# compbioproj-cdna-to-genome-map-align/gmap-2024

Measured on AMD Instinct MI355X. Metric: aligned cDNA reads/sec (2 kb, GRCh38) at 1/2/4/8 MI355X; DP HBM GB/s vs peak, higher is better.
Workload: dtype int32

## Files before the change

gmap-2024_amd/csrc/gmapdp_engine.cpp:

```cpp
#include <dlfcn.h>
#include <hip/hip_runtime.h>
#include <time.h>
#include <unistd.h>

#include <algorithm>
#include <climits>
#include <cctype>
#include <cstdio>
#include <cstdlib>
#include <cstring>
#include <map>
#include <memory>
#include <condition_variable>
#include <mutex>
#include <thread>
#include <atomic>
#include <sys/mman.h>
#include <string>
#include <tuple>
#include <utility>
#include <vector>

#include "gmapdp_internal.h"
#include "me_device.h"
// ... 841 lines not shown
  if (!T) return GMAPDP_EINVAL;
  hipError_t e = ctx->din.ensure(16 * n);
  if (e == hipSuccess) e = ctx->dout.ensure(n);
  if (e != hipSuccess) return fail(ctx, GMAPDP_ENOMEM, "canonical-link buffers: %s", e);
  unsigned char* din = (unsigned char*)ctx->din.p;
  hipStream_t s = ctx->stream;
  e = hipMemcpyAsync(din, prevpos, 8 * n, hipMemcpyHostToDevice, s);
  if (e == hipSuccess) e = hipMemcpyAsync(din + 8 * n, currpos, 8 * n, hipMemcpyHostToDevice, s);
  if (e == hipSuccess)
    e = launch_canon_links((long long)n, s, ctx->d_genome, ctx->genome_words, T, (const gmapdp_coord_t*)din,
                           (const gmapdp_coord_t*)(din + 8 * n), plusp, chroffset, chrhigh, (uint8_t*)ctx->dout.p);
  if (e == hipSuccess) e = hipMemcpyAsync(out, ctx->dout.p, n, hipMemcpyDeviceToHost, s);
  if (e == hipSuccess) e = ctx_sync(ctx, s);
  return e == hipSuccess ? GMAPDP_OK : fail(ctx, GMAPDP_ELAUNCH, "canonical links: %s", e);
}

}

static const size_t kLdsBudget = 64 * 1024;
static size_t env_size(const char* name, size_t dflt);
static size_t dpx_lds_dirs_max() {
  static const size_t v = env_size("GMAPDP_DPX_LDS_DIRS_MAX", 4 * 1024);
  return v;
}

static int pick_R(int W) {
  int R = 1;
  while (R * 64 < W) R <<= 1;
  return R;
}

static size_t lds_bucket(size_t lds) {
  static const size_t b[] = {4096, 8192, 16384, 32768, 49152, 65536, 98304, 163840};
  for (size_t x : b)
    if (lds <= x) return x;
  return lds;
}

static size_t gg_lds_bucket(size_t lds) {
  static const size_t b[] = {4096,  6144,  8192,  10240, 12288, 14336, 16384, 20480, 24576,
                             28672, 32768, 40960, 49152, 65536, 98304, 163840};
  for (size_t x : b)
    if (lds <= x) return x;
  return lds;
}

static size_t env_size(const char* name, size_t dflt) {
  const char* e = getenv(name);
  return e ? (size_t)strtoull(e, nullptr, 10) : dflt;
}

static size_t gg_lds_dirs_max() { return env_size("GMAPDP_GG_LDS_DIRS_MAX", 0); }
static bool gg_rowfill() { return env_size("GMAPDP_GG_ROWFILL", 1) != 0; }
static bool rows_disabled() {
  static const bool v = env_size("GMAPDP_DP_ROWS", 1) == 0;
  return v;
}
static size_t latency_batch() {
  static const size_t v = env_size("GMAPDP_LATENCY_BATCH", 1024);
  return v;
}

static size_t slot_bucket(size_t b) {
  static const size_t s[] = {256, 384, 512, 768, 1024, 1536, 2048, 3072, 4096, 6144, 8192, 12288, 16384};
  for (size_t x : s)
    if (b <= x) return x;
  return 0;
}

static void null_result(gmapdp_result& res, int score, int dpi) {
  res.npairs = 0;
  res.traceback_score = score;
  res.nmatches = res.nmismatches = res.nopens = res.nindels = 0;
  res.dynprogindex = dpi;
}

static int next_dpi(int dpi) { return dpi + (dpi > 0 ? 1 : -1); }

static int convert_single(const gmapdp_ctx* ctx, const gmapdp_single_problem& p, gmapdp_result& res, DevProblem& d) {
  if (p.rlength <= 0 || p.glength <= 0 || p.rlength > GMAPDP_MAX_RLENGTH || p.glength > GMAPDP_MAX_GLENGTH) {
    null_result(res, GMAPDP_NEG_INFINITY_32, next_dpi(p.dynprogindex));
    return 0;
  }
  std::memset(&d, 0, sizeof(d));
  d.kind = kSingle;
  d.qbase = p.qoff;
  d.rlength = p.rlength;
  d.glength = p.glength;
  d.roffset = p.roffset;
  d.goffset = p.goffset;
  d.chroffset = p.chroffset;
  d.chrhigh = p.chrhigh;
  const double dr = p.defect_rate;
  d.mismatchtype = dr < 0.003 ? kHighQ : (dr < 0.014 ? kMedQ : kLowQ);
  if (ctx->user_dynprog_p) {
    d.open = ctx->user_open;
    d.extend = ctx->user_extend;
  } else if (dr < 0.003) {
    d.open = -8; d.extend = -3;
  } else if (dr < 0.014) {
    d.open = -7; d.extend = -2;
  } else {
    d.open = -6; d.extend = -1;
  }
  const bool watson = p.flags & GMAPDP_WATSON;
  d.flags = (watson ? kFWatson : 0) | ((p.flags & GMAPDP_JUMP_LATE) ? kFLate : 0) |
// ... 1903 lines not shown
struct OligoClasses {
  std::vector<int> key;
  std::vector<size_t> slots;
  std::map<int, std::vector<int>> classes;
};
static const int kBuckets[] = {1024, 2048, 4096, 8192, 16384};

static int oligo_classify(gmapdp_ctx* ctx, const gmapdp_oligo_problem* problems, int n, const char* qseq_uc,
                          size_t qbytes, bool major_only, OligoClasses& C) {
  std::vector<int> distinct(n, 0);
  std::vector<const char*> rej(n, nullptr);
  plan_parallel((size_t)n, plan_threads((size_t)n * 128), [&](size_t lo, size_t hi, int) {
    std::vector<uint32_t> bm(2048, 0u);
    for (size_t i = lo; i < hi; i++) {
      const gmapdp_oligo_problem& p = problems[i];
      if (major_only && p.minor)
        rej[i] = "Stage2_scan takes the major oligoindex only (minor must be 0)";
      else if (p.querylength <= 8)
        rej[i] = "stage-2 seeding needs querylength > 8 (Oligoindex_set_inquery)";
      else if (p.qoff < 0 || (size_t)p.qoff + (size_t)p.querylength > qbytes)
        rej[i] = "query outside the arena";
      else
        distinct[i] = oligo_distinct(qseq_uc + p.qoff, p.querylength, bm);
    }
  });
  C.key.resize(n);
  C.slots.resize(n);
  for (int i = 0; i < n; i++) {
    const gmapdp_oligo_problem& p = problems[i];
    if (rej[i]) return bad(ctx, rej[i]);
    const uint64_t win = oligo_window(p);
    if (win > 0) {
      const uint64_t lpl = (uint64_t)p.chroffset + p.chrend + (p.plusp ? 0 : 1) - 8;
      const uint64_t h = (lpl >> 4) + 1;
      if (3 * (h >> 1) + 1 >= ctx->genome_words) return bad(ctx, "stage-2 window past the genome");
    }
    if (distinct[i] > kOligoMaxDistinct && !ctx->long_queries)
      return bad(ctx, "query with more than 16384 distinct 8-mers");
    if (distinct[i] > kOligoMaxDistinct) {
      C.key[i] = kOligoLongKey;
      ctx->long_calls.fetch_add(1, std::memory_order_relaxed);
    } else {
      int umax = kBuckets[0];
      for (int b : kBuckets)
        if (distinct[i] <= b) { umax = b; break; }
      C.key[i] = 2 * umax + (win >= 65536 ? 1 : 0);
    }
    C.slots[i] = oligo_pool_slots(p);
    C.classes[C.key[i]].push_back(i);
  }
  return GMAPDP_OK;
}

static void oligo_dev_problem(DevOligoProblem& d, const gmapdp_oligo_problem& p, int umax, int mode) {
  std::memset(&d, 0, sizeof(d));
  d.querylength = p.querylength;
  d.chrstart = p.chrstart;
  d.chrend = p.chrend;
  d.chroffset = p.chroffset;
  d.chrhigh = p.chrhigh;
  d.plusp = p.plusp ? 1 : 0;
  d.minor = p.minor ? 1 : 0;
  d.umax = umax;
  d.reduce = oi_reduction_of(mode, p.plusp != 0);
}

extern "C" {

size_t gmapdp_oligo_positions_capacity(const gmapdp_oligo_problem* problems, int n) {
  size_t c = 0;
  for (int i = 0; i < n; i++) c += oligo_table_cap(problems[i]);
  return c;
}
size_t gmapdp_oligo_diagonal_capacity(const gmapdp_oligo_problem* problems, int n) {
  size_t c = 0;
  for (int i = 0; i < n; i++) c += oligo_diag_cap(problems[i]);
  return c;
}

}

struct gmapdp_oligo_plan {
  int n = 0;
  DevMem<DevOligoProblem> d_probs;
  DevMem<unsigned char> d_scratch;
  std::vector<std::pair<int, int>> launches;
  std::vector<int> umax;
  std::vector<int> keys;
  size_t table_cap = 0, diag_cap = 0, scratch_cap = 0;
  DevMem<int32_t> d_nhits;
  bool split = false;
  DevMem<uint64_t> d_pool;
  DevMem<unsigned long long> d_pool_counter;
  unsigned long long pool_cap = 0;
  bool sizing = false;
  std::vector<DevOligoProblem> ord;
  int mode = 0;
};

static constexpr int kOligoChunkProblems = 16384;
static constexpr size_t kOligoChunkBytes = size_t(3) << 30;
static constexpr size_t kOligoSizingChunkBytes = size_t(32) << 30;

static void oligo_layout(gmapdp_oligo_plan* P, const std::vector<size_t>& slots, bool fallback,
                         const std::vector<size_t>& tcap, const std::vector<size_t>& dcap, bool local,
                         const std::vector<size_t>* hcap = nullptr) {
  P->launches.clear();
  P->umax.clear();
  P->scratch_cap = 0;
  P->pool_cap = 0;
  P->table_cap = 0;
  P->diag_cap = 0;
  size_t cb = 0, cs = 0, ct = 0, cd = 0;
  int first = 0;
  auto close = [&](int end) {
    if (end > first) {
      P->launches.push_back({first, end - first});
// ... 33 lines not shown
}

static hipError_t oligo_buffers(gmapdp_ctx* ctx, gmapdp_oligo_plan* P) {
  const int n = P->n;
  hipError_t e = hipSuccess;
  if (P->split || P->sizing) {
    const bool t = P->sizing;
    e = ctx->oprobs.ensure(sizeof(DevOligoProblem) * std::max(n, 1));
    if (e == hipSuccess) e = ctx->oscratch.ensure(std::max<size_t>(P->scratch_cap, 256), t);
    if (e == hipSuccess) e = ctx->opool.ensure(sizeof(uint64_t) * std::max<size_t>(P->pool_cap, 1), t);
    if (e == hipSuccess) e = ctx->opoolctr.ensure(sizeof(unsigned long long));
    P->d_probs.view((DevOligoProblem*)ctx->oprobs.p);
    P->d_scratch.view((unsigned char*)ctx->oscratch.p);
    P->d_pool.view((uint64_t*)ctx->opool.p);
    P->d_pool_counter.view((unsigned long long*)ctx->opoolctr.p);
    if (e == hipSuccess && n)
      e = hipMemcpyAsync(P->d_probs, P->ord.data(), sizeof(DevOligoProblem) * n, hipMemcpyHostToDevice, ctx->stream);
    return e;
  }
  P->d_scratch.reset();
  P->d_pool.reset();
  if (!P->d_probs.owns()) e = P->d_probs.alloc(sizeof(DevOligoProblem) * std::max(n, 1));
  if (e == hipSuccess) e = P->d_scratch.alloc(std::max<size_t>(P->scratch_cap, 256));
  if (e == hipSuccess) e = P->d_pool.alloc(sizeof(uint64_t) * std::max<size_t>(P->pool_cap, 1));
  if (e == hipSuccess && !P->d_pool_counter.owns()) e = P->d_pool_counter.alloc(sizeof(unsigned long long));
  if (e == hipSuccess && n)
    e = hipMemcpy(P->d_probs, P->ord.data(), sizeof(DevOligoProblem) * n, hipMemcpyHostToDevice);
  return e;
}

static int oligo_plan_build(gmapdp_ctx* ctx, const gmapdp_oligo_problem* problems, int n, const char* qseq_uc,
                            size_t qbytes, std::unique_ptr<gmapdp_oligo_plan>& plan, bool split,
                            bool sizing = false) {
  plan.reset();
  if (const int rc_alt = refuse_alt(ctx, "stage-2 seeding (gmapdp_oligo_*, gmapdp_stage2_*)")) return rc_alt;
  if (oi_reduction_of(ctx->mode, true) < 0)
    return bad(ctx, "stage 2 in a non-stranded cmet / atoi / ttoc mode (GMAP supports the stranded modes only)");
  if (!ctx->d_genome) return GMAPDP_ENOGENOME;
  (void)hipSetDevice(ctx->device);
  OligoClasses C;
  if (int rc = oligo_classify(ctx, problems, n, qseq_uc, qbytes, false, C)) return rc;
  std::vector<size_t> tcap(n), dcap(n);
  for (int i = 0; i < n; i++) {
    tcap[i] = oligo_table_cap(problems[i]);
    dcap[i] = oligo_diag_cap(problems[i]);
  }
  std::unique_ptr<gmapdp_oligo_plan> P(new gmapdp_oligo_plan());
  P->n = n;
  P->mode = ctx->mode;
  P->split = split;
  P->sizing = sizing;
  P->ord.resize(n);
  P->keys.reserve(n);
  for (auto& kv : C.classes)
    for (int i : kv.second) {
      DevOligoProblem& d = P->ord[P->keys.size()];
      oligo_dev_problem(d, problems[i], kv.first >> 1, ctx->mode);
      d.qoff = problems[i].qoff;
      d.index = i;
      P->keys.push_back(kv.first);
    }
  oligo_layout(P.get(), C.slots, !sizing, tcap, dcap, sizing);
  if (const char* ev = std::getenv("GMAPDP_OLIGO_POOL_SLOTS")) P->pool_cap = std::strtoull(ev, nullptr, 10);
  const hipError_t e = oligo_buffers(ctx, P.get());
  if (e != hipSuccess) return fail(ctx, GMAPDP_ENOMEM, "oligo plan: %s", e);
  plan = std::move(P);
  return GMAPDP_OK;
}

static hipError_t oligo_plan_relayout(gmapdp_ctx* ctx, gmapdp_oligo_plan* P, const gmapdp_oligo_problem* problems,
                                      const gmapdp_oligo_result* ores, const int32_t* nhits) {
  const int n = P->n;
  std::vector<size_t> slots(n), tcap(n), dcap(n), hcap(n);
  for (int i = 0; i < n; i++) {
    const size_t tp = (size_t)std::max(ores[i].totalpositions, 0);
    tcap[i] = std::min<size_t>(oligo_table_cap(problems[i]), tp);
    dcap[i] = ores[i].oned_matrix_p < 0 ? oligo_diag_cap(problems[i]) : (size_t)std::max(ores[i].ndiagonals, 0);
    slots[i] = 3 * tp;
    hcap[i] = (size_t)std::max(nhits[i], 0);
  }
  {
    std::vector<int> key(n), idx(n);
    for (int k = 0; k < n; k++) {
      const int i = P->ord[k].index;
      key[k] = (P->keys[k] & 1) && !oligo_key_long(P->keys[k]) && nhits[i] >= 0 && nhits[i] < 65536 ? P->keys[k] - 1
                                                                                                     : P->keys[k];
      idx[k] = k;
    }
    std::stable_sort(idx.begin(), idx.end(), [&](int a, int b) { return key[a] < key[b]; });
    std::vector<DevOligoProblem> ord(n);
    std::vector<int> keys(n);
    for (int k = 0; k < n; k++) {
      ord[k] = P->ord[idx[k]];
      keys[k] = key[idx[k]];
    }
    P->ord.swap(ord);
    P->keys.swap(keys);
  }
  oligo_layout(P, slots, false, tcap, dcap, false, &hcap);
  P->sizing = false;
  P->d_nhits.reset();
  return oligo_buffers(ctx, P);
}

extern "C" {

int gmapdp_oligo_plan_create(gmapdp_ctx* ctx, const gmapdp_oligo_problem* problems, int n, const char* qseq_uc,
                             size_t qbytes, gmapdp_oligo_plan** plan) {
  if (!ctx || !plan || n < 0 || (n > 0 && (!problems || !qseq_uc))) return GMAPDP_EINVAL;
  std::unique_ptr<gmapdp_oligo_plan> p;
// ... 90 lines not shown
  }
  e = hipMemcpyAsync(results, ctx->oresults.p, sizeof(gmapdp_oligo_result) * n, hipMemcpyDeviceToHost, s);
  if (e == hipSuccess) e = hipMemcpyAsync(npositions, ctx->onpos.p, sizeof(int32_t) * qbytes, hipMemcpyDeviceToHost, s);
  if (e == hipSuccess) e = hipMemcpyAsync(mappings, ctx->omap.p, sizeof(int32_t) * qbytes, hipMemcpyDeviceToHost, s);
  if (e == hipSuccess && toff)
    e = hipMemcpyAsync(positions, ctx->otable.p, sizeof(uint32_t) * toff, hipMemcpyDeviceToHost, s);
  if (e == hipSuccess && doff)
    e = hipMemcpyAsync(diagonals, ctx->odiag.p, 4 * sizeof(int32_t) * doff, hipMemcpyDeviceToHost, s);
  if (e == hipSuccess) e = ctx_sync(ctx, s);
  if (e != hipSuccess) return fail(ctx, GMAPDP_ELAUNCH, "oligo execution: %s", e);
  oligo_absolute_mappings(problems, n, results, mappings);
  return GMAPDP_OK;
}

}

struct ScanLaunch {
  int first = 0, count = 0, key = 0;
  unsigned long long pool_slots = 0;
  size_t scratch = 0, pool = 0, table = 0, diag = 0, quc = 0, npos = 0, map = 0, ores = 0, total = 0;
};
struct gmapdp_scan_plan {
  int n = 0, mode = 0;
  DevMem<DevOligoProblem> d_probs;
  DevMem<unsigned char> d_extra;
  DevMem<unsigned char> d_arena;
  size_t arena_bytes = 0, budget = 0;
  std::vector<ScanLaunch> launches;
};

static constexpr size_t kScanBudgetFloor = size_t(8) << 30;

static size_t scan_budget(gmapdp_ctx* ctx) {
  if (const char* ev = std::getenv("GMAPDP_SCAN_ARENA_MB")) return (size_t)std::strtoull(ev, nullptr, 10) << 20;
  size_t held = 0;
  for (const DevBuf* b : {&ctx->oscratch, &ctx->opool, &ctx->otable, &ctx->odiag, &ctx->onpos, &ctx->omap})
    held += b->cap;
  return std::max(held, kScanBudgetFloor);
}

extern "C" {

int gmapdp_scan_plan_create(gmapdp_ctx* ctx, const gmapdp_oligo_problem* problems, int n, const char* qseq_uc,
                            size_t qbytes, gmapdp_scan_plan** plan) {
  if (!ctx || !plan || n < 0 || (n > 0 && (!problems || !qseq_uc))) return GMAPDP_EINVAL;
  *plan = nullptr;
  if (oi_reduction_of(ctx->mode, true) < 0)
    return bad(ctx, "stage 2 in a non-stranded cmet / atoi / ttoc mode (GMAP supports the stranded modes only)");
  if (const int rc_alt = refuse_alt(ctx, "Stage2_scan (gmapdp_scan_plan_*)")) return rc_alt;
  if (!ctx->d_genome) return GMAPDP_ENOGENOME;
  (void)hipSetDevice(ctx->device);
  OligoClasses C;
  if (int rc = oligo_classify(ctx, problems, n, qseq_uc, qbytes,  true, C)) return rc;
  std::unique_ptr<gmapdp_scan_plan> P(new gmapdp_scan_plan());
  P->n = n;
  P->mode = ctx->mode;
  P->budget = scan_budget(ctx);
  struct Extra { int32_t src_qoff, out_index; };
  std::vector<DevOligoProblem> ord;
  std::vector<Extra> extra;
  ord.reserve(n);
  extra.reserve(n);
  size_t cs = 0, cp = 0, ct = 0, cd = 0, cq = 0;
  ScanLaunch L;
  auto close = [&]() {
    if (L.count == 0) return;
    size_t off = 0;
    auto carve = [&](size_t bytes) { const size_t at = off; off = align_up(off + bytes, 256); return at; };
    L.scratch = carve(cs);
    L.pool = carve(sizeof(uint64_t) * cp);
    L.table = carve(sizeof(uint32_t) * ct);
    L.diag = carve(4 * sizeof(int32_t) * cd);
    L.quc = carve(cq);
    L.npos = carve(sizeof(int32_t) * cq);
    L.map = carve(sizeof(int32_t) * cq);
    L.ores = carve(sizeof(gmapdp_oligo_result) * (size_t)L.count);
    L.total = off;
    L.pool_slots = cp;
    P->arena_bytes = std::max(P->arena_bytes, off);
    P->launches.push_back(L);
    L = ScanLaunch();
    L.first = (int)ord.size();
    cs = cp = ct = cd = cq = 0;
  };
  for (auto& kv : C.classes)
    for (int i : kv.second) {
      const gmapdp_oligo_problem& p = problems[i];
      const uint32_t w = p.chrend > p.chrstart ? p.chrend - p.chrstart : 0;
      const size_t lt = oligo_key_long(kv.first) ? scratch_bytes_oi_long() : 0;
      const size_t mb = lt + align_up(scratch_bytes_oi(p.querylength, w), 256);
      const size_t fb = align_up(scratch_bytes_oi_fallback(p.querylength, w), 256);
      const size_t tcap = oligo_table_cap(p), dcap = oligo_diag_cap(p);
      const size_t slots = C.slots[i];
      const size_t qpad = align_up((size_t)p.querylength, 16);
      const size_t bytes = mb + fb + 8 * slots + 4 * tcap + 16 * dcap + 9 * qpad + sizeof(gmapdp_oligo_result) + 8 * 256;
      const size_t open = cs + 8 * cp + 4 * ct + 16 * cd + 9 * cq + sizeof(gmapdp_oligo_result) * (size_t)L.count + 8 * 256;
      if (L.count > 0 && (kv.first != L.key || L.count >= kOligoChunkProblems || open + bytes > P->budget ||
                          cq + qpad > 0x7fffffffull))
        close();
      if (L.count == 0) L.key = kv.first;
      DevOligoProblem d;
      oligo_dev_problem(d, p, kv.first >> 1, ctx->mode);
      d.qoff = (int32_t)cq;
      d.index = L.count;
      d.table_offset = (int64_t)ct;
      d.diag_offset = (int64_t)cd;
      d.scratch_offset = (int64_t)(cs + lt);
      d.fallback_offset = (int64_t)(cs + mb);
      d.hit_cap = (uint32_t)std::min<size_t>((size_t)w + 2, 0xffffffffu);
      d.table_cap = (uint32_t)std::min<size_t>(tcap, 0xffffffffu);
      d.diag_cap = (uint32_t)std::min<size_t>(dcap, 0xffffffffu);
      ord.push_back(d);
      extra.push_back(Extra{p.qoff, i});
      cs += mb + fb;
      cp += slots;
      ct += tcap;
      cd += dcap;
      cq += qpad;
      L.count++;
    }
  close();
  hipError_t e = hipSuccess;
  if (n) {
    e = P->d_probs.alloc(sizeof(DevOligoProblem) * (size_t)n);
    if (e == hipSuccess) e = P->d_extra.alloc(sizeof(Extra) * (size_t)n);
    if (e == hipSuccess) e = P->d_arena.alloc(P->arena_bytes + 256);
    if (e == hipSuccess) e = hipMemcpy(P->d_probs, ord.data(), sizeof(DevOligoProblem) * (size_t)n, hipMemcpyHostToDevice);
    if (e == hipSuccess) e = hipMemcpy(P->d_extra, extra.data(), sizeof(Extra) * (size_t)n, hipMemcpyHostToDevice);
  }
  if (e != hipSuccess) return fail(ctx, GMAPDP_ENOMEM, "scan plan: %s", e);
  *plan = P.release();
  return GMAPDP_OK;
}

int gmapdp_scan_plan_nlaunches(const gmapdp_scan_plan* plan) { return plan ? (int)plan->launches.size() : 0; }
size_t gmapdp_scan_plan_scratch_bytes(const gmapdp_scan_plan* plan) { return plan ? plan->arena_bytes : 0; }
void gmapdp_scan_plan_destroy(gmapdp_scan_plan* plan) { delete plan; }

int gmapdp_scan_plan_run(gmapdp_ctx* ctx, const gmapdp_scan_plan* plan, const char* d_qseq_uc,
                         gmapdp_scan_result* d_results, void* stream) {
  if (!ctx || !plan) return GMAPDP_EINVAL;
  if (const int rc_alt = refuse_alt(ctx, "Stage2_scan (gmapdp_scan_plan_*)")) return rc_alt;
  if (plan->mode != ctx->mode) return bad(ctx, "a scan plan made by a context of another mode");
  if (plan->n == 0) return GMAPDP_OK;
  if (!d_qseq_uc || !d_results) return GMAPDP_EINVAL;
  (void)hipSetDevice(ctx->device);
  hipStream_t s = stream_of(ctx, stream);
  unsigned char* A = plan->d_arena;
  unsigned long long* pool_counter = reinterpret_cast<unsigned long long*>(A + plan->arena_bytes);
  int32_t* flag = reinterpret_cast<int32_t*>(A + plan->arena_bytes + 64);
  if (hipMemsetAsync(flag, 0, sizeof(int32_t), s) != hipSuccess)
    return fail(ctx, GMAPDP_ELAUNCH, "scan flag reset: %s", hipGetLastError());
  for (const ScanLaunch& L : plan->launches) {
    const hipError_t e = launch_s2scan(
        L.key & 1, plan->mode != 0, oligo_key_long(L.key), L.count, lds_bytes_oi(L.key >> 1, L.key & 1), s, plan->d_probs + L.first,
// ... 964 lines not shown
```

gmap-2024_amd/csrc/gmapdp_internal.h:

```cpp
#pragma once
#include <stdint.h>

namespace gmapdp {

constexpr int kNegInf32 = -32768;
constexpr int kMatch = 1, kMismatch = -3, kQopen = -3, kQindel = -1, kTopen = -3, kTindel = -1;
constexpr int kMicrointronLength = 9;
constexpr int kMaxR = 64;

enum GClass : uint8_t { kA = 0, kC = 1, kG = 2, kT = 3, kN = 4, kStar = 5 };
constexpr int kNClass = 8;

enum Kind : int32_t { kSingle = 0, kEnd5 = 1, kEnd3 = 2 };
enum Endalign : int32_t { kQueryendGap = 0, kQueryendIndels = 1, kQueryendNogaps = 2, kBestLocal = 3 };

constexpr int32_t kFWatson = 0x1;
constexpr int32_t kFLate = 0x2;
constexpr int32_t kFRequirePos = 0x4;
constexpr int32_t kFSegLeft = 0x8;
constexpr int32_t kFSegRevcomp = 0x10;
constexpr int32_t kFRev = 0x20;
constexpr int32_t kFScoreUC = 0x40;
constexpr int32_t kFSimd = 0x80;

// ... 83 lines not shown
  uint64_t chrhigh;
  uint64_t segpos, segbound;
  uint64_t rsegpos, rsegbound;
  int32_t open;
  int32_t extend;
  int32_t mismatchtype;
  int32_t flags;
  int32_t genestrand;
  int32_t dynprogindex;
  int32_t pair_offset;
  int64_t scratch_offset;
};

constexpr int kMismatchEndQ = 3;
constexpr int kFullMatch = 3;
struct DevSjProblem {
  int32_t qbase;
  int32_t jbase;
  int32_t rlength;
  int32_t glength;
  int32_t roffset;
  int32_t goffset_anchor;
  int32_t goffset_far;
  int32_t known_jump;
  int32_t contlength;
  int32_t lband;
  int32_t uband;
  int32_t open;
  int32_t extend;
  int32_t late;
  int32_t end3p;
  int32_t genestrand;
  int32_t dynprogindex;
  int32_t pair_offset;
  int32_t simd;
  int64_t dirs_offset;
};

struct DevOligoProblem {
  int32_t qoff;
  int32_t querylength;
  uint32_t chrstart, chrend;
  uint64_t chroffset, chrhigh;
  int32_t plusp;
  int32_t minor;
  int32_t umax;
  int32_t index;
  int64_t table_offset;
  int64_t diag_offset;
  int64_t scratch_offset;
  int64_t fallback_offset;
  uint32_t hit_cap, table_cap, diag_cap;
  int32_t reduce;
};

struct DevStage2Problem {
  int32_t qoff;
  int32_t querylength;
  uint32_t chrstart, chrend;
  uint64_t chroffset, chrhigh;
  int32_t plusp;
  int32_t splicingp;
  uint32_t maxintronlen;
  int32_t index;
  int64_t scratch_offset;
  int32_t kind;
  int32_t query_offset;
};

}
```

gmap-2024_amd/csrc/oi_kernel.hip:

```cpp
#include <cstdlib>

#include "dp_device.h"
#include "oi_reduce.h"

namespace gmapdp {

constexpr int kOiK = 8;

#ifdef GMAPDP_OI_TIMING
__device__ unsigned long long g_oi_marks[2][16];
__device__ unsigned int g_oi_wave[3][16384];
#define OI_MARK(k)                                                 \
  do {                                                             \
    if (threadIdx.x == 0) {                                        \
      atomicAdd(&g_oi_marks[0][k], (unsigned long long)wall_clock64()); \
      atomicAdd(&g_oi_marks[1][k], 1ull);                          \
    }                                                              \
  } while (0)
#else
#define OI_MARK(k) \
  do {             \
  } while (0)
#endif
constexpr int kOiWords = 65536 / 32;
// ... 428 lines not shown
                        }
                        const uint64_t cm = ballot(c);
                        if (c) evA[C + lanes_below(cm, lane)] = key;
                        oi_hist_add(lane, c, di, D, hist);
                        C += __popcll(cm);
                      });
    __threadfence_block();
    oi_wave_sync();
    OI_MARK(5);
    const K* S = oi_radix<KT>(lane, evA, evB, C, D, hist);
    OI_MARK(6);
    uint64_t* gkey = sizeof(K) == 8 ? reinterpret_cast<uint64_t*>(S == evA ? evB : evA) : pool + base + E;
    int maxn = 0;
    const int ngood = oi_sweep<KT>(lane, S, C, qlen, nq, lookback, suffn, cum, grec, gkey, good, gcap, maxn);
    if (filtered && ngood != -1 && (ngood == 0 || maxn < suffn)) {
      filtered = false;
      continue;
    }
    ngood_out = ngood;
    maxn_out = maxn;
    return true;
  }
}

template <typename CT>
__device__ __forceinline__ void count_inc(CT* cnt, int u) {
  if constexpr (sizeof(CT) == 4) {
    atomicAdd(reinterpret_cast<uint32_t*>(cnt) + u, 1u);
  } else {
    atomicAdd(reinterpret_cast<uint32_t*>(cnt) + (u >> 1), 1u << (16 * (u & 1)));
  }
}

__device__ void oi_report_overflow(const DevOligoProblem& P, int tid, int nthreads, int qlen, int32_t* npq,
                                   int32_t* mpq, gmapdp_oligo_result* results, unsigned char* poolslot) {
  for (int i = tid; i < qlen; i += nthreads) {
    npq[i] = 0;
    mpq[i] = -1;
  }
  if (tid == 0) {
    gmapdp_oligo_result res;
    res.totalpositions = 0;
    res.maxnconsecutive = 0;
    res.oned_matrix_p = -1;
    res.ndiagonals = 0;
    res.table_offset = P.table_offset;
    res.diag_offset = P.diag_offset;
    results[P.index] = res;
    *reinterpret_cast<unsigned long long*>(poolslot) = ~0ull;
  }
}

constexpr int kOiWaves = 2;
#ifdef GMAPDP_OI_STAGE
constexpr bool kOiStage = true;
#else
constexpr bool kOiStage = false;
#endif

constexpr int kOiLongIds = 65536;
constexpr size_t kOiLongTableBytes = 2 * sizeof(uint32_t) * (size_t)kOiLongIds;
__device__ __forceinline__ void oi_long_sync() {
  __builtin_amdgcn_fence(__ATOMIC_SEQ_CST, "wavefront");
  __builtin_amdgcn_s_waitcnt(0);
  __builtin_amdgcn_wave_barrier();
}
template <bool kLong, typename CT>
__device__ __forceinline__ uint32_t oi_tab(const CT* p) {
  if constexpr (kLong) return __hip_atomic_load(p, __ATOMIC_RELAXED, __HIP_MEMORY_SCOPE_AGENT);
  else return (uint32_t)*p;
}

#define OI_PASS_ARGS                                                                                          \
  const DevOligoProblem *__restrict__ probs, const uint32_t *__restrict__ blocks, const char *__restrict__ quc_all, \
      unsigned char *__restrict__ scratch, gmapdp_oligo_result *__restrict__ results,                             \
      int32_t *__restrict__ npos_out, int32_t *__restrict__ map_out, uint32_t *__restrict__ table_all,            \
      unsigned long long *__restrict__ pool_counter, unsigned long long pool_cap, int32_t *__restrict__ nhits_out
template <typename CT, bool kModal, bool kLong = false>
__device__ __forceinline__ void oi_pass(OI_PASS_ARGS) {
  static_assert(!kLong || sizeof(CT) == 4, "the long class counts in 32 bits");
  extern __shared__ __attribute__((aligned(16))) unsigned char smem[];
  __shared__ int nh_wave[kOiWaves];
  const int tid = threadIdx.x, lane = tid & 63;
  const int wave = __builtin_amdgcn_readfirstlane(tid >> 6);
  const DevOligoProblem P = probs[blockIdx.x];
  uint32_t* bitmap = reinterpret_cast<uint32_t*>(smem);
  uint16_t* wrank = reinterpret_cast<uint16_t*>(smem + 4 * kOiWords);
  CT* cnt = kLong ? reinterpret_cast<CT*>(scratch + P.scratch_offset - kOiLongTableBytes)
                  : reinterpret_cast<CT*>(smem + 6 * kOiWords);
  CT* offs = cnt + P.umax;
  const char* quc = quc_all + P.qoff;
  const int qlen = P.querylength;
  OI_MARK(0);
#ifdef GMAPDP_OI_TIMING
  const unsigned long long oi_t0 = wall_clock64();
#endif
  const int nq = qlen - kOiK + 1;

  for (int w = tid; w < kOiWords; w += 64 * kOiWaves) bitmap[w] = 0u;
  __syncthreads();
  int32_t* npq = npos_out + P.qoff;
  int32_t* mpq = map_out + P.qoff;
  for (int sb = 4 * 64 * wave; sb < qlen; sb += 4 * 64 * kOiWaves) {
    int ch[5];
#pragma unroll
    for (int r = 0; r < 5; r++) {
      const int i = sb + 64 * r + lane;
      ch[r] = i < qlen ? nt_code(quc[i]) : -1;
    }
#pragma unroll
    for (int r = 0; r < 4; r++) {
      const int i = sb + 64 * r + lane;
      uint32_t m = 0;
      bool ok = i < nq;
#pragma unroll
      for (int j = 0; j < kOiK; j++) {
        const int src = (lane + j) & 63;
        const int a = __shfl(ch[r], src, 64), b = __shfl(ch[r + 1], src, 64);
        const int cj = lane + j < 64 ? a : b;
        ok = ok && cj >= 0;
        m = (m << 2) | ((uint32_t)cj & 3u);
      }
      if (i < qlen) {
        mpq[i] = ok ? (int)m : -1;
        npq[i] = 0;
      }
      if (ok) atomicOr(&bitmap[m >> 5], 1u << (m & 31));
    }
  }
  __syncthreads();
  int run = 0;
  for (int base = 0; base < kOiWords; base += 64) {
    const int c = __popc(bitmap[base + lane]);
    const int incl = wave_scan_add(lane, c);
    if (wave == 0) wrank[base + lane] = (uint16_t)(run + incl - c);
// ... 45 lines not shown
      } else {
        vv = ~v;
      }
      auto oligo_at = [&](int j) -> uint32_t {
        return (uint32_t)(vv >> (P.plusp ? 2 * (24 - j) : 2 * j)) & 0xFFFFu;
      };
      uint32_t vmask = 0;
      if (h <= hhi) {
        const uint64_t p0 = 16 * h;
        const int jlo = left > p0 ? (int)(left - p0) : 0;
        const int jhi = lpl < p0 + 15 ? (int)(lpl - p0) : 15;
        if (jlo <= jhi) vmask = (0xFFFFu >> (15 - jhi)) & (0xFFFFu << jlo);
      }
      uint32_t hm = 0;
#pragma unroll
      for (int j = 0; j < 16; j++) {
        const uint32_t m = oligo_at(j);
        hm |= ((bitmap[m >> 5] >> (m & 31)) & 1u) << j;
      }
      hm &= vmask;
      const int c = __popc(hm);
      const int incl = wave_scan_add(lane, c);
      int o = nhits + incl - c;
      for (uint32_t r = hm; r; r &= r - 1) {
        const int j = __ffs(r) - 1;
        const uint32_t m = oligo_at(j);
        bool in;
        const int id = oligo_id(bitmap, wrank, m, in);
        count_inc(cnt, id);
        if ((uint32_t)o < P.hit_cap) {
          const uint32_t at = wave ? P.hit_cap - 1 - (uint32_t)o : (uint32_t)o;
          const uint32_t k = (uint32_t)(16 * h + j - left);
          if (compact) hitlist32[at] = (k << kIdShift) | (uint32_t)id;
          else hitlist[at] = make_uint2(k, (uint32_t)id);
        }
        o++;
      }
      nhits += __builtin_amdgcn_readlane(incl, 63);
    };
    for (uint64_t hb0 = hlo; hlo <= hhi && hb0 <= hhi; hb0 += 64 * kOiAhead) {
#pragma unroll
      for (int a = 0; a < kOiAhead; a++) {
        const uint64_t hb = hb0 + 64 * a;
        if (hb > hhi) break;
        const uint64_t v = (uint64_t)pw0[a] | ((uint64_t)pw1[a] << 32);
        const uint64_t hh = hb + 64 * kOiAhead + lane;
        pw0[a] = hh <= hhi ? half_word(blocks, hh) : 0u;
        pw1[a] = hh <= hhi ? half_word(blocks, hh + 1) : 0u;
        step(hb, v);
      }
    }
  }
  if (lane == 0) nh_wave[wave] = nhits;
  if constexpr (kLong) __threadfence();
  __syncthreads();
  const int n0 = nh_wave[0], n1 = nh_wave[1];
  nhits = n0 + n1;
  if (nhits_out && tid == 0) nhits_out[P.index] = nhits;
  for (int u = tid; u < U; u += 64 * kOiWaves) cnt[u] = (CT)(oi_tab<kLong>(&cnt[u]) & 255u);
  if constexpr (kLong) __threadfence();
  __syncthreads();
  __shared__ uint32_t tot_s;
  const int idbits = U > 1 ? 32 - __clz(U - 1) : 1;
  int* cum = reinterpret_cast<int*>(base_s);
  int totalpositions = 0;
  if (wave == 0) {
    uint32_t tot = 0;
    int cumrun = 0;
    for (int sb = 0; sb < nq; sb += 4 * 64) {
      int mm[4];
#pragma unroll
      for (int r = 0; r < 4; r++) {
        const int i = sb + 64 * r + lane;
        mm[r] = i < nq ? mpq[i] : -1;
      }
#pragma unroll
      for (int r = 0; r < 4; r++) {
        if (sb + 64 * r >= nq) break;
        const int i = sb + 64 * r + lane;
        int id = -1;
        uint32_t cv = 0;
        if (mm[r] >= 0) {
          bool in;
          id = oligo_id(bitmap, wrank, (uint32_t)mm[r], in);
          cv = oi_tab<kLong>(&cnt[id]);
        }
        const bool cand = id >= 0 && (cv >> 8) == 0u;
        uint64_t eq = ballot(cand);
        for (int b = 0; b < idbits; b++) {
          const uint64_t m = ballot((id >> b) & 1);
          eq &= ((id >> b) & 1) ? m : ~m;
        }
        const bool first = cand && lanes_below(eq, lane) == 0;
        const uint32_t kept = cv & 255u;
        const uint32_t c = first ? kept : 0u;
        const uint32_t incl = (uint32_t)wave_scan_add(lane, (int)c);
        if (first) {
          offs[id] = (CT)(tot + incl - c);
          cnt[id] = (CT)(cv | 0x100u);
        }
        tot += (uint32_t)__builtin_amdgcn_readlane((int)incl, 63);
        if constexpr (kLong) oi_long_sync();
        else oi_wave_sync();
        int nh = -1;
        if (i < nq) {
          int mo = -1;
          if (id >= 0) {
            nh = (int)kept;
            npq[i] = nh;
            if (nh > 0) mo = (int32_t)oi_tab<kLong>(&offs[id]);
          }
          mpq[i] = mo;
        }
        const int cincl = wave_scan_add(lane, nh == 0 ? 1 : 0);
        if (i < nq) cum[i] = cumrun + cincl;
        cumrun += __builtin_amdgcn_readlane(cincl, 63);
        totalpositions += __builtin_amdgcn_readlane(wave_scan_add(lane, nh > 0 ? nh : 0), 63);
      }
    }
    if (lane == 0) tot_s = tot;
  }
  __syncthreads();
  const uint32_t tot = tot_s;
  OI_MARK(2);
  if ((uint32_t)nhits > P.hit_cap || tot > P.table_cap || (sizeof(CT) == 2 && nhits > 65535)) {
    oi_report_overflow(P, tid, 64 * kOiWaves, qlen, npq, mpq, results, base_s + so.poolbase);
    return;
  }

  uint32_t* table = table_all + P.table_offset;
  uint32_t* slotarr = hitlist32 + P.hit_cap;
  const uint32_t chrpos0 = P.plusp ? P.chrstart : (P.chrhigh - P.chroffset) - P.chrend;
  __threadfence_block();
  constexpr int kP2 = 4;
  uint32_t at_n[kP2];
  uint2 hv_n[kP2];
  auto load_hits = [&](int c0) {
#pragma unroll
    for (int r = 0; r < kP2; r++) {
      const int sl = c0 + 64 * r + lane;
      at_n[r] = 0;
      hv_n[r] = make_uint2(0u, 0xFFFFFFFFu);
      if (wave == 0 && sl < nhits) {
        const int a = P.plusp ? nhits - 1 - sl : sl;
        const uint32_t at = a < n0 ? (uint32_t)a : P.hit_cap - 1 - (uint32_t)(a - n0);
        at_n[r] = at;
        if (compact) {
          const uint32_t e = hitlist32[at];
          hv_n[r] = make_uint2(e >> kIdShift, e & ((1u << kIdShift) - 1u));
        } else {
          hv_n[r] = hitlist[at];
        }
      }
    }
  };
  load_hits(0);
  for (int c0 = 0; wave == 0 && c0 < nhits; c0 += 64 * kP2) {
    uint32_t at_c[kP2];
    uint2 hv_c[kP2];
#pragma unroll
    for (int r = 0; r < kP2; r++) {
      at_c[r] = at_n[r];
      hv_c[r] = hv_n[r];
    }
    load_hits(c0 + 64 * kP2);
#pragma unroll
    for (int r = 0; r < kP2; r++) {
      if (c0 + 64 * r >= nhits) break;
      const uint32_t at = at_c[r], k = hv_c[r].x;
      const int id = (int)hv_c[r].y;
      const uint64_t hits = ballot(id >= 0);
      uint64_t eq = hits;
      for (int b = 0; b < idbits; b++) {
        const uint64_t m = ballot((id >> b) & 1);
        eq &= ((id >> b) & 1) ? m : ~m;
      }
      if (id >= 0) {
        const int rank = lanes_below(eq, lane);
        const int same = __popcll(eq);
        const uint32_t cv = oi_tab<kLong>(&cnt[id]);
        const int r0 = (int)(cv & 255u);
        const uint32_t slot = oi_tab<kLong>(&offs[id]) + (uint32_t)(r0 - rank - 1);
        if (kOiStage && !kLong && compact)
          slotarr[at] = r0 - rank > 0 ? slot : 0xFFFFFFFFu;
        else if (r0 - rank > 0)
          table[slot] = chrpos0 + (P.plusp ? k : (uint32_t)(npos - 1) - k);
        if (rank == 0) cnt[id] = (CT)(cv - (uint32_t)min(same, r0));
      }
      if constexpr (kLong) oi_long_sync();
    }
  }
  __threadfence_block();
  __syncthreads();
  if (kOiStage && !kLong && compact) {
    uint32_t* stage = reinterpret_cast<uint32_t*>(smem);
    constexpr uint32_t kStage = 6 * kOiWords / 4;
    for (uint32_t b0 = 0; b0 < tot; b0 += kStage) {
      for (int a = tid; a < nhits; a += 64 * kOiWaves) {
        const uint32_t at = a < n0 ? (uint32_t)a : P.hit_cap - 1 - (uint32_t)(a - n0);
        const uint32_t sd = slotarr[at] - b0;
        if (sd < kStage) {
          const uint32_t k = hitlist32[at] >> 14;
          stage[sd] = chrpos0 + (P.plusp ? k : (uint32_t)(npos - 1) - k);
        }
      }
      __syncthreads();
      const uint32_t nb = min(kStage, tot - b0);
      for (uint32_t j = tid; j < nb; j += 64 * kOiWaves) table[b0 + j] = stage[j];
      __syncthreads();
    }
  }
  OI_MARK(3);
  __threadfence_block();
  __syncthreads();
  if (wave) return;

  gmapdp_oligo_result res;
  res.totalpositions = totalpositions;
  res.maxnconsecutive = 0;
  res.oned_matrix_p = 0;
  res.ndiagonals = 0;
  res.table_offset = P.table_offset;
  res.diag_offset = P.diag_offset;
  __threadfence_block();
  if (lane == 0) {
    results[P.index] = res;
    unsigned long long b = ~0ull;
    if (P.chrend > P.chrstart) {
      const unsigned long long need = 3ull * (unsigned long long)totalpositions;
      b = atomicAdd(pool_counter, need);
      if (b + need > pool_cap) b = ~0ull;
    }
    *reinterpret_cast<unsigned long long*>(base_s + so.poolbase) = b;
  }
  OI_MARK(4);
#ifdef GMAPDP_OI_TIMING
  if (lane == 0 && P.index < 16384) g_oi_wave[0][P.index] = (unsigned int)(wall_clock64() - oi_t0);
#endif
}

__device__ bool oi_mappings_walk(int lane, const DevOligoProblem& P, unsigned char* __restrict__ scratch, int qlen,
                                 int nq, const int32_t* __restrict__ npq, const int32_t* __restrict__ mpq,
                                 const int* __restrict__ cum, const uint32_t* __restrict__ table, uint32_t chrinit,
                                 int diag_lookback, int suffn, int32_t* __restrict__ good, int& ngood_out,
                                 int& maxn_out) {
  if (P.fallback_offset < 0) return false;
  const ScratchOiFb fb = scratch_oi_fb(qlen, P.chrend - P.chrstart);
  unsigned char* initp = scratch + P.fallback_offset + fb.initp;
  OiState* st = reinterpret_cast<OiState*>(scratch + P.fallback_offset + fb.states);
  for (size_t b = 16 * (size_t)lane; b < fb.states - fb.initp; b += 16 * 64)
    *reinterpret_cast<uint4*>(initp + b) = make_uint4(0u, 0u, 0u, 0u);
  __threadfence_block();
  int best = -1;
  int ngood = 0, maxn = 0;
  for (int cb = 0; cb < nq; cb += 64) {
    const int qi = cb + lane;
    int c_nh = 0, c_mo = 0, c_cum = 0;
    uint32_t c_h0 = 0;
    if (qi < nq) {
      c_nh = npq[qi];
      c_mo = mpq[qi];
      c_cum = cum[qi];
      if (c_nh > 0) c_h0 = table[c_mo];
    }
    const int cend = min(64, nq - cb);
    for (int j = 0; j < cend; j++) {
      const int nh = __builtin_amdgcn_readlane(c_nh, j);
// ... 747 lines not shown
```

Measured before the change: 384,000.

## Scatter oligo table entries from both waves with LDS atomic counters

Adds a two-wave scatter path for the oligo index table fill. Each wave walks its own half of the hit list, one wave counting up from the low end and the other down from the high end, using packed 8-bit counters in LDS updated with atomics. This replaces the single-wave serial scatter and spreads the work across both wavefronts. It also removes the compile-time LDS staging path and one extra block barrier. The new path falls back to the old single-wave loop when a counter overflowed past 255, or when the GMAPDP_OI_PASS2 environment variable is set to 0. It adds atomic contention, and its ordering correctness depends on the low/high counter split.

```diff
diff --git a/gmap-2024_amd/csrc/gmapdp_engine.cpp b/gmap-2024_amd/csrc/gmapdp_engine.cpp
--- a/gmap-2024_amd/csrc/gmapdp_engine.cpp
+++ b/gmap-2024_amd/csrc/gmapdp_engine.cpp
@@ -917,6 +917,7 @@
 
 static size_t gg_lds_dirs_max() { return env_size("GMAPDP_GG_LDS_DIRS_MAX", 0); }
 static bool gg_rowfill() { return env_size("GMAPDP_GG_ROWFILL", 1) != 0; }
+static bool oi_pass2() { return env_size("GMAPDP_OI_PASS2", 1) != 0; }
 static bool rows_disabled() {
   static const bool v = env_size("GMAPDP_DP_ROWS", 1) == 0;
   return v;
@@ -2926,7 +2927,7 @@
   return GMAPDP_OK;
 }
 
-static void oligo_dev_problem(DevOligoProblem& d, const gmapdp_oligo_problem& p, int umax, int mode) {
+static void oligo_dev_problem(DevOligoProblem& d, const gmapdp_oligo_problem& p, int umax, int mode, bool pass2) {
   std::memset(&d, 0, sizeof(d));
   d.querylength = p.querylength;
   d.chrstart = p.chrstart;
@@ -2937,6 +2938,7 @@
   d.minor = p.minor ? 1 : 0;
   d.umax = umax;
   d.reduce = oi_reduction_of(mode, p.plusp != 0);
+  d.flags = pass2 ? kOiPass2 : 0;
 }
 
 extern "C" {
@@ -3076,10 +3078,11 @@
   P->sizing = sizing;
   P->ord.resize(n);
   P->keys.reserve(n);
+  const bool pass2 = oi_pass2();
   for (auto& kv : C.classes)
     for (int i : kv.second) {
       DevOligoProblem& d = P->ord[P->keys.size()];
-      oligo_dev_problem(d, problems[i], kv.first >> 1, ctx->mode);
+      oligo_dev_problem(d, problems[i], kv.first >> 1, ctx->mode, pass2);
       d.qoff = problems[i].qoff;
       d.index = i;
       P->keys.push_back(kv.first);
@@ -3276,6 +3279,7 @@
   (void)hipSetDevice(ctx->device);
   OligoClasses C;
   if (int rc = oligo_classify(ctx, problems, n, qseq_uc, qbytes,  true, C)) return rc;
+  const bool pass2 = oi_pass2();
   std::unique_ptr<gmapdp_scan_plan> P(new gmapdp_scan_plan());
   P->n = n;
   P->mode = ctx->mode;
@@ -3324,7 +3328,7 @@
         close();
       if (L.count == 0) L.key = kv.first;
       DevOligoProblem d;
-      oligo_dev_problem(d, p, kv.first >> 1, ctx->mode);
+      oligo_dev_problem(d, p, kv.first >> 1, ctx->mode, pass2);
       d.qoff = (int32_t)cq;
       d.index = L.count;
       d.table_offset = (int64_t)ct;
diff --git a/gmap-2024_amd/csrc/gmapdp_internal.h b/gmap-2024_amd/csrc/gmapdp_internal.h
--- a/gmap-2024_amd/csrc/gmapdp_internal.h
+++ b/gmap-2024_amd/csrc/gmapdp_internal.h
@@ -159,7 +159,9 @@
   int64_t fallback_offset;
   uint32_t hit_cap, table_cap, diag_cap;
   int32_t reduce;
+  int32_t flags;
 };
+constexpr int32_t kOiPass2 = 1;
 
 struct DevStage2Problem {
   int32_t qoff;
diff --git a/gmap-2024_amd/csrc/oi_kernel.hip b/gmap-2024_amd/csrc/oi_kernel.hip
--- a/gmap-2024_amd/csrc/oi_kernel.hip
+++ b/gmap-2024_amd/csrc/oi_kernel.hip
@@ -504,11 +504,6 @@
 }
 
 constexpr int kOiWaves = 2;
-#ifdef GMAPDP_OI_STAGE
-constexpr bool kOiStage = true;
-#else
-constexpr bool kOiStage = false;
-#endif
 
 constexpr int kOiLongIds = 65536;
 constexpr size_t kOiLongTableBytes = 2 * sizeof(uint32_t) * (size_t)kOiLongIds;
@@ -533,6 +528,7 @@
   static_assert(!kLong || sizeof(CT) == 4, "the long class counts in 32 bits");
   extern __shared__ __attribute__((aligned(16))) unsigned char smem[];
   __shared__ int nh_wave[kOiWaves];
+  __shared__ int wrap_s;
   const int tid = threadIdx.x, lane = tid & 63;
   const int wave = __builtin_amdgcn_readfirstlane(tid >> 6);
   const DevOligoProblem P = probs[blockIdx.x];
@@ -684,12 +680,19 @@
     }
   }
   if (lane == 0) nh_wave[wave] = nhits;
+  if (tid == 0) wrap_s = 0;
   if constexpr (kLong) __threadfence();
   __syncthreads();
   const int n0 = nh_wave[0], n1 = nh_wave[1];
   nhits = n0 + n1;
   if (nhits_out && tid == 0) nhits_out[P.index] = nhits;
-  for (int u = tid; u < U; u += 64 * kOiWaves) cnt[u] = (CT)(oi_tab<kLong>(&cnt[u]) & 255u);
+  bool wrapped = false;
+  for (int u = tid; u < U; u += 64 * kOiWaves) {
+    const uint32_t c = oi_tab<kLong>(&cnt[u]);
+    wrapped |= c > 255u;
+    cnt[u] = (CT)(c & 255u);
+  }
+  if (wrapped) wrap_s = 1;
   if constexpr (kLong) __threadfence();
   __syncthreads();
   __shared__ uint32_t tot_s;
@@ -761,22 +764,83 @@
   }
 
   uint32_t* table = table_all + P.table_offset;
-  uint32_t* slotarr = hitlist32 + P.hit_cap;
   const uint32_t chrpos0 = P.plusp ? P.chrstart : (P.chrhigh - P.chroffset) - P.chrend;
   __threadfence_block();
   constexpr int kP2 = 4;
-  uint32_t at_n[kP2];
+  const bool both = !kLong && (P.flags & kOiPass2) && wrap_s == 0;
+  if constexpr (!kLong) {
+    if (both) {
+      for (int u = tid; u < U; u += 64 * kOiWaves) cnt[u] = (CT)((cnt[u] & 255u) << 8);
+      __syncthreads();
+      const bool up = (wave == 0) == (P.plusp != 0);
+      const int nw = wave ? n1 : n0;
+      const uint32_t a0 = wave ? P.hit_cap - (uint32_t)n1 : 0u;
+      uint2 hv_n[kP2];
+      auto load_own = [&](int c0) {
+#pragma unroll
+        for (int r = 0; r < kP2; r++) {
+          const int s = c0 + 64 * r + lane;
+          hv_n[r] = make_uint2(0u, 0xFFFFFFFFu);
+          if (s < nw) {
+            if (compact) {
+              const uint32_t e = hitlist32[a0 + (uint32_t)s];
+              hv_n[r] = make_uint2(e >> kIdShift, e & ((1u << kIdShift) - 1u));
+            } else {
+              hv_n[r] = hitlist[a0 + (uint32_t)s];
+            }
+          }
+        }
+      };
+      load_own(0);
+      for (int c0 = 0; c0 < nw; c0 += 64 * kP2) {
+        uint2 hv_c[kP2];
+#pragma unroll
+        for (int r = 0; r < kP2; r++) hv_c[r] = hv_n[r];
+        load_own(c0 + 64 * kP2);
+        uint32_t pre[kP2], old[kP2], of[kP2];
+#pragma unroll
+        for (int r = 0; r < kP2; r++) {
+          const int id = (int)hv_c[r].y;
+          pre[r] = old[r] = of[r] = 0u;
+          if (id >= 0) {
+            uint32_t* w = reinterpret_cast<uint32_t*>(cnt) + (sizeof(CT) == 2 ? id >> 1 : id);
+            const int sh = sizeof(CT) == 2 ? 16 * (id & 1) : 0;
+            pre[r] = __hip_atomic_load(w, __ATOMIC_RELAXED, __HIP_MEMORY_SCOPE_WORKGROUP) >> sh;
+            old[r] = (up ? atomicAdd(w, 1u << sh) : atomicSub(w, 0x100u << sh)) >> sh;
+            of[r] = (uint32_t)offs[id];
+          }
+        }
+#pragma unroll
+        for (int r = 0; r < kP2; r++) {
+          const int id = (int)hv_c[r].y;
+          const uint32_t k = hv_c[r].x;
+          const int lo = (int)(pre[r] & 255u), hi = (int)((pre[r] >> 8) & 255u);
+          const int mine = up ? lo : hi;
+          int rank = 0;
+          if (ballot(id >= 0 && mine != (int)((old[r] >> (up ? 0 : 8)) & 255u))) {
+            uint64_t eq = ballot(id >= 0);
+            for (int b = 0; b < idbits; b++) {
+              const uint64_t m = ballot((id >> b) & 1);
+              eq &= ((id >> b) & 1) ? m : ~m;
+            }
+            rank = lanes_below(eq, lane);
+          }
+          const int ord = up ? lo + rank : hi - 1 - rank;
+          if (id >= 0 && (up ? ord < hi : ord >= lo))
+            table[of[r] + (uint32_t)ord] = chrpos0 + (P.plusp ? k : (uint32_t)(npos - 1) - k);
+        }
+      }
+    }
+  }
   uint2 hv_n[kP2];
   auto load_hits = [&](int c0) {
 #pragma unroll
     for (int r = 0; r < kP2; r++) {
       const int sl = c0 + 64 * r + lane;
-      at_n[r] = 0;
       hv_n[r] = make_uint2(0u, 0xFFFFFFFFu);
-      if (wave == 0 && sl < nhits) {
+      if (wave == 0 && !both && sl < nhits) {
         const int a = P.plusp ? nhits - 1 - sl : sl;
         const uint32_t at = a < n0 ? (uint32_t)a : P.hit_cap - 1 - (uint32_t)(a - n0);
-        at_n[r] = at;
         if (compact) {
           const uint32_t e = hitlist32[at];
           hv_n[r] = make_uint2(e >> kIdShift, e & ((1u << kIdShift) - 1u));
@@ -787,19 +851,15 @@
     }
   };
   load_hits(0);
-  for (int c0 = 0; wave == 0 && c0 < nhits; c0 += 64 * kP2) {
-    uint32_t at_c[kP2];
+  for (int c0 = 0; wave == 0 && !both && c0 < nhits; c0 += 64 * kP2) {
     uint2 hv_c[kP2];
 #pragma unroll
-    for (int r = 0; r < kP2; r++) {
-      at_c[r] = at_n[r];
-      hv_c[r] = hv_n[r];
-    }
+    for (int r = 0; r < kP2; r++) hv_c[r] = hv_n[r];
     load_hits(c0 + 64 * kP2);
 #pragma unroll
     for (int r = 0; r < kP2; r++) {
       if (c0 + 64 * r >= nhits) break;
-      const uint32_t at = at_c[r], k = hv_c[r].x;
+      const uint32_t k = hv_c[r].x;
       const int id = (int)hv_c[r].y;
       const uint64_t hits = ballot(id >= 0);
       uint64_t eq = hits;
@@ -813,9 +873,7 @@
         const uint32_t cv = oi_tab<kLong>(&cnt[id]);
         const int r0 = (int)(cv & 255u);
         const uint32_t slot = oi_tab<kLong>(&offs[id]) + (uint32_t)(r0 - rank - 1);
-        if (kOiStage && !kLong && compact)
-          slotarr[at] = r0 - rank > 0 ? slot : 0xFFFFFFFFu;
-        else if (r0 - rank > 0)
+        if (r0 - rank > 0)
           table[slot] = chrpos0 + (P.plusp ? k : (uint32_t)(npos - 1) - k);
         if (rank == 0) cnt[id] = (CT)(cv - (uint32_t)min(same, r0));
       }
@@ -824,27 +882,7 @@
   }
   __threadfence_block();
   __syncthreads();
-  if (kOiStage && !kLong && compact) {
-    uint32_t* stage = reinterpret_cast<uint32_t*>(smem);
-    constexpr uint32_t kStage = 6 * kOiWords / 4;
-    for (uint32_t b0 = 0; b0 < tot; b0 += kStage) {
-      for (int a = tid; a < nhits; a += 64 * kOiWaves) {
-        const uint32_t at = a < n0 ? (uint32_t)a : P.hit_cap - 1 - (uint32_t)(a - n0);
-        const uint32_t sd = slotarr[at] - b0;
-        if (sd < kStage) {
-          const uint32_t k = hitlist32[at] >> 14;
-          stage[sd] = chrpos0 + (P.plusp ? k : (uint32_t)(npos - 1) - k);
-        }
-      }
-      __syncthreads();
-      const uint32_t nb = min(kStage, tot - b0);
-      for (uint32_t j = tid; j < nb; j += 64 * kOiWaves) table[b0 + j] = stage[j];
-      __syncthreads();
-    }
-  }
   OI_MARK(3);
-  __threadfence_block();
-  __syncthreads();
   if (wave) return;
 
   gmapdp_oligo_result res;
```

Result: faster. 388,600 (median of 4 runs) (+1.2%).
